# shaderko/velocity-asr

Measured on AMD Instinct MI355X. Metric: audio-sec/sec (RTFx) + frames/s, 5M model batch=32×10s @ 1/2/4/8 MI355X, higher is better.
Workload: dtype f32

## Files before the change

### include/vasr.h

```cpp
#ifndef VASR_H_
#define VASR_H_

#include <stdint.h>

#ifdef __cplusplus
extern "C" {
#endif

#define VASR_ABI_VERSION 21

#define VASR_OK 0
#define VASR_EINVAL (-1)
#define VASR_EUNSUPPORTED (-2)

int vasr_version(void);
const char* vasr_last_error(void);

enum vasr_option {
    VASR_OPT_SCAN_LANES = 0,
    VASR_OPT_SCAN_CHUNK = 1,
    VASR_OPT_TAIL_ROWS = 2,
    VASR_OPT_GEMM_ENGINE = 3,
    VASR_OPT_TAIL_WAVES = 4,
    VASR_OPT_SCAN_SPLIT = 5,
// ... 93 lines not shown

int vasr_ssm_tree_bwd_f32(const float* x, int64_t ld_x, const float* z, int64_t ld_z,
                          const float* dt, int64_t ld_dt, const float* bc, int64_t ld_bc,
                          const float* A, const float* A2, const float* D,
                          const float* g, int64_t ld_g,
                          float* dx, float* ddt, float* dz, float* dB, float* dC,
                          float* dA_part, float* dD_part, float* workspace, int64_t workspace_floats,
                          int B, int L, int Di, int N, void* stream);
int64_t vasr_ssm_tree_bwd_workspace_floats(int B, int L, int Di, int N);

int vasr_ssm_block_tail_f32(const float* g, int64_t ldg, const float* x, int64_t ldx, const uint16_t* wo16,
                            const float* ln_w, const float* ln_b, float ln_eps, const uint16_t* w1_16,
                            const float* b1, const uint16_t* w2_16, const float* b2, float* out, int64_t ldo,
                            int M, int D, int E, void* stream);
int vasr_ssm_block_tail_gated_f32(const float* yd, int64_t ldy, const float* u, int64_t ldu, const uint16_t* wz,
                                  int mode, const float* x, int64_t ldx, const uint16_t* wo16,
                                  const float* ln_w, const float* ln_b, float ln_eps, const uint16_t* w1_16,
                                  const float* b1, const uint16_t* w2_16, const float* b2, float* out, int64_t ldo,
                                  int M, int D, int E, void* stream);
int vasr_ssm_block_tail_bf16(const float* g, int64_t ldg, const float* x, int64_t ldx, const uint16_t* wo16,
                             const float* ln_w, const float* ln_b, float ln_eps, const uint16_t* w1_16,
                             const float* b1, const uint16_t* w2_16, const float* b2, float* out, int64_t ldo,
                             int M, int D, int E, void* stream);
int vasr_ssm_block_tail_gated_bf16(const float* yd, int64_t ldy, const float* u, int64_t ldu, const uint16_t* wz,
                                   int mode, const float* x, int64_t ldx, const uint16_t* wo16,
                                   const float* ln_w, const float* ln_b, float ln_eps, const uint16_t* w1_16,
                                   const float* b1, const uint16_t* w2_16, const float* b2, float* out, int64_t ldo,
                                   int M, int D, int E, void* stream);
int vasr_pack_weights16_bf16(const uint16_t* W, int64_t ldw, int N, int K, uint16_t* out, void* stream);
int64_t vasr_pack_weights16_bf16_elems(int N, int K);
int vasr_split_weights16_bf16x3(const float* W, int64_t ldw, int N, int K, uint16_t* out, void* stream);
int64_t vasr_split_weights16_elems(int N, int K);

int vasr_flac_decode(const uint8_t* data, int64_t n, float* out, int64_t out_cap, int* channels,
                     int* sample_rate, int* bits, int64_t* samples);
int64_t vasr_resample_length(int64_t n, int orig_sr, int new_sr);
int vasr_resample_f32(const float* x, int channels, int64_t n, int64_t ld_x, int orig_sr, int new_sr,
                      float* y, int64_t ld_y);

int vasr_reflect_pad_f32(const float* audio, int64_t ld_audio, float* xp, int64_t ld_out,
                         int B, int S, int pad, void* stream);
int vasr_mel_log_norm_f32(const float* power, int64_t ld_power, int64_t stride_power,
                          const int32_t* fb_rowptr, const int32_t* fb_col, const float* fb_val,
                          float* out, int64_t out_stride, int frame_off, int B, int F, int n_mels,
                          int normalize, float* workspace, void* stream);
int vasr_mel_log_norm_var_f32(const float* power, int64_t ld_power, int64_t stride_power,
                              const int32_t* fb_rowptr, const int32_t* fb_col, const float* fb_val,
                              float* out, int64_t out_stride, int frame_off, int B, int F, int n_mels,
                              int normalize, const int32_t* frames, float* workspace, void* stream);
int64_t vasr_mel_workspace_floats(int B, int F, int n_mels);

int vasr_stft_power_400_f32(const float* audio, int64_t ld_audio, int B, int S, const float* window,
                            float* power, int64_t ldp, int64_t stride_power, void* stream);
int vasr_stft_power_400_var_f32(const float* audio, int64_t ld_audio, int B, int S, const int32_t* samples,
                                const float* window, float* power, int64_t ldp, int64_t stride_power,
                                void* stream);
int vasr_pad_frames_f32(const float* x, float* out, int out_frames, int off,
                        int B, int F, int C, void* stream);

int vasr_adaptive_pool_f32(const float* x, float* out, int B, int L, int C, int K, void* stream);
int vasr_adaptive_pool_var_f32(const float* x, float* out, int B, int L, int C, int K, const int32_t* lens,
                               const int32_t* ks, void* stream);

int vasr_ln_adaptive_pool_f32(const float* x, const float* w, const float* b, float eps, float* out, int B, int L,
                              int C, int K, const int32_t* lens, const int32_t* ks, void* stream);

// ... 72 lines not shown
```

### velocity-asr_amd/velocity_asr/_lib.py

```python

from __future__ import annotations

import ctypes
import os
import re
from typing import Optional

import torch

ABI_VERSION = 21
_HERE = os.path.dirname(os.path.abspath(__file__))
LIB_PATH = os.environ.get("VASR_LIB") or os.path.join(_HERE, "lib", "libvasr_hip.so")
HEADER_PATH = os.path.normpath(os.path.join(_HERE, "..", "..", "include", "vasr.h"))

(EPI_NONE, EPI_GELU, EPI_SOFTPLUS_FROM, EPI_RESIDUAL, EPI_GELU_PE, EPI_PAIR_POWER, EPI_PAIR_FUSION,
 EPI_ARGMAX) = range(8)
OPT_SCAN_LANES, OPT_SCAN_CHUNK, OPT_TAIL_ROWS, OPT_GEMM_ENGINE, OPT_TAIL_WAVES, OPT_SCAN_SPLIT, OPT_DW_ROWS = range(7)

c_i32, c_i64, c_f32, c_p = ctypes.c_int32, ctypes.c_int64, ctypes.c_float, ctypes.c_void_p


class GemmArgs(ctypes.Structure):

    _fields_ = [
# ... 28 lines not shown
    "vasr_add_table_f32": ([c_p, c_p, c_p, ctypes.c_int, ctypes.c_int, ctypes.c_int, c_p], ctypes.c_int),
    "vasr_ln_dwconv_prenorm_f32": ([c_p, c_p, c_p, c_f32, c_p, c_p, c_p, c_p, c_p, c_p] + [ctypes.c_int] * 4
                                   + [c_f32, c_p], ctypes.c_int),
    "vasr_ln_dwconv_f32": ([c_p, c_p, c_p, c_p, c_p, c_p] + [ctypes.c_int] * 4 + [c_f32, c_p], ctypes.c_int),
    "vasr_ssm_scan_f32": ([c_p, c_i64, c_p, c_i64, c_p, c_i64, c_p, c_p, c_p, c_i64] + [ctypes.c_int] * 5 + [c_p],
                          ctypes.c_int),
    "vasr_ssm_scan_chunked_f32": ([c_p, c_i64, c_p, c_i64, c_p, c_i64, c_p, c_p, c_p, c_i64] + [ctypes.c_int] * 5
                                  + [c_p, c_i64, c_p], ctypes.c_int),
    "vasr_ssm_scan_ungated_f32": ([c_p, c_i64, c_p, c_i64, c_p, c_i64, c_p, c_p, c_p, c_i64] + [ctypes.c_int] * 5 + [c_p],
                                  ctypes.c_int),
    "vasr_ssm_scan_workspace_floats": ([ctypes.c_int] * 4, c_i64),
    "vasr_ssm_scan_save_f32": ([c_p, c_i64, c_p, c_i64, c_p, c_i64, c_p, c_p, c_p, c_i64] + [ctypes.c_int] * 5
                               + [c_p, c_i64, c_p], ctypes.c_int),
    "vasr_ssm_scan_checkpoint_floats": ([ctypes.c_int] * 4, c_i64),
    "vasr_ssm_scan_bwd_f32": ([c_p, c_i64, c_p, c_i64, c_p, c_i64, c_p, c_i64, c_p, c_p, c_p, c_p, c_i64] + [c_p] * 9
                              + [c_i64] + [ctypes.c_int] * 4 + [c_p], ctypes.c_int),
    "vasr_ssm_scan_bwd_workspace_floats": ([ctypes.c_int] * 4, c_i64),
    "vasr_ssm_tree_bwd_f32": ([c_p, c_i64, c_p, c_i64, c_p, c_i64, c_p, c_i64, c_p, c_p, c_p, c_p, c_i64] + [c_p] * 8
                              + [c_i64] + [ctypes.c_int] * 4 + [c_p], ctypes.c_int),
    "vasr_ssm_tree_bwd_workspace_floats": ([ctypes.c_int] * 4, c_i64),
    "vasr_ssm_scan_split_selected": ([ctypes.c_int] * 4, ctypes.c_int),
    "vasr_ssm_block_tail_f32": ([c_p, c_i64, c_p, c_i64, c_p, c_p, c_p, c_f32, c_p, c_p, c_p, c_p, c_p, c_i64]
                                + [ctypes.c_int] * 3 + [c_p], ctypes.c_int),
    "vasr_ssm_block_tail_gated_f32": ([c_p, c_i64, c_p, c_i64, c_p, ctypes.c_int, c_p, c_i64, c_p, c_p, c_p, c_f32, c_p,
                                       c_p, c_p, c_p, c_p, c_i64] + [ctypes.c_int] * 3 + [c_p], ctypes.c_int),
    "vasr_ssm_block_tail_gated_bf16": ([c_p, c_i64, c_p, c_i64, c_p, ctypes.c_int, c_p, c_i64, c_p, c_p, c_p, c_f32, c_p,
                                        c_p, c_p, c_p, c_p, c_i64] + [ctypes.c_int] * 3 + [c_p], ctypes.c_int),
    "vasr_ssm_block_tail_bf16": ([c_p, c_i64, c_p, c_i64, c_p, c_p, c_p, c_f32, c_p, c_p, c_p, c_p, c_p, c_i64]
                                 + [ctypes.c_int] * 3 + [c_p], ctypes.c_int),
    "vasr_pack_weights16_bf16": ([c_p, c_i64, ctypes.c_int, ctypes.c_int, c_p, c_p], ctypes.c_int),
    "vasr_pack_weights16_bf16_elems": ([ctypes.c_int, ctypes.c_int], c_i64),
    "vasr_split_weights16_bf16x3": ([c_p, c_i64, ctypes.c_int, ctypes.c_int, c_p, c_p], ctypes.c_int),
    "vasr_split_weights16_elems": ([ctypes.c_int, ctypes.c_int], c_i64),
    "vasr_flac_decode": ([c_p, c_i64, c_p, c_i64, c_p, c_p, c_p, c_p], ctypes.c_int),
    "vasr_resample_length": ([c_i64, ctypes.c_int, ctypes.c_int], c_i64),
    "vasr_resample_f32": ([c_p, ctypes.c_int, c_i64, c_i64, ctypes.c_int, ctypes.c_int, c_p, c_i64], ctypes.c_int),
    "vasr_reflect_pad_f32": ([c_p, c_i64, c_p, c_i64, ctypes.c_int, ctypes.c_int, ctypes.c_int, c_p], ctypes.c_int),
    "vasr_mel_log_norm_f32": ([c_p, c_i64, c_i64, c_p, c_p, c_p, c_p, c_i64] + [ctypes.c_int] * 5 + [c_p, c_p],
                              ctypes.c_int),
    "vasr_mel_workspace_floats": ([ctypes.c_int] * 3, c_i64),
    "vasr_stft_power_400_f32": ([c_p, c_i64, ctypes.c_int, ctypes.c_int, c_p, c_p, c_i64, c_i64, c_p], ctypes.c_int),
    "vasr_stft_power_400_var_f32": ([c_p, c_i64, ctypes.c_int, ctypes.c_int, c_p, c_p, c_p, c_i64, c_i64, c_p],
                                    ctypes.c_int),
    "vasr_mel_log_norm_var_f32": ([c_p, c_i64, c_i64, c_p, c_p, c_p, c_p, c_i64] + [ctypes.c_int] * 5 + [c_p, c_p, c_p],
                                  ctypes.c_int),
    "vasr_adaptive_pool_var_f32": ([c_p, c_p] + [ctypes.c_int] * 4 + [c_p, c_p, c_p], ctypes.c_int),
    "vasr_pooled_attention_var_f32": ([c_p, c_i64, c_p, c_p] + [ctypes.c_int] * 5 + [c_p, c_p], ctypes.c_int),
    "vasr_ctc_collapse_var": ([c_p, ctypes.c_int, ctypes.c_int, c_p, ctypes.c_int, ctypes.c_int, c_p, c_p, c_p, c_p,
                               c_p], ctypes.c_int),
    "vasr_pad_frames_f32": ([c_p, c_p] + [ctypes.c_int] * 5 + [c_p], ctypes.c_int),
    "vasr_ln_adaptive_pool_f32": ([c_p, c_p, c_p, c_f32, c_p] + [ctypes.c_int] * 4 + [c_p, c_p, c_p], ctypes.c_int),
    "vasr_adaptive_pool_f32": ([c_p, c_p] + [ctypes.c_int] * 4 + [c_p], ctypes.c_int),
    "vasr_pooled_attention_f32": ([c_p, c_i64, c_p, c_p] + [ctypes.c_int] * 5 + [c_p], ctypes.c_int),
    "vasr_pooled_attention_bwd_f32": ([c_p, c_i64, c_p, c_p, c_p, c_p, c_p, c_i64] + [ctypes.c_int] * 5 + [c_p, c_p],
                                      ctypes.c_int),
    "vasr_pooled_attention_bwd_workspace_floats": ([ctypes.c_int] * 5, c_i64),
    "vasr_adaptive_pool_bwd_f32": ([c_p, c_p] + [ctypes.c_int] * 4 + [c_p, c_p, c_p], ctypes.c_int),
    "vasr_argmax_f32": ([c_p, c_i64, ctypes.c_int, ctypes.c_int, c_p, c_p], ctypes.c_int),
    "vasr_fakequant_f32": ([c_p, c_i64, c_p, c_i64, ctypes.c_int, ctypes.c_int, c_p, c_p, ctypes.c_int, c_f32, c_f32,
                            c_p], ctypes.c_int),
    "vasr_minmax_f32": ([c_p, c_i64, ctypes.c_int, ctypes.c_int, c_p, c_p, c_p], ctypes.c_int),
    "vasr_argmax_keys": ([c_p, c_i64, ctypes.c_int, ctypes.c_int, c_p, c_p], ctypes.c_int),
    "vasr_ctc_collapse_keys": ([c_p, c_i64] + [ctypes.c_int] * 3 + [c_p, ctypes.c_int, ctypes.c_int] + [c_p] * 6,
                               ctypes.c_int),
    "vasr_ctc_beam_search": ([c_p, c_i64, c_i64] + [ctypes.c_int] * 5 + [c_p] * 5 + [c_p], ctypes.c_int),
    "vasr_ctc_beam_workspace_elems": ([ctypes.c_int, ctypes.c_int], c_i64),
# ... 65 lines not shown
```

### velocity-asr_amd/velocity_asr/attention.py

```python

from __future__ import annotations

import math
import os
from typing import Optional, Sequence, Tuple

import torch
import torch.nn as nn

from . import _lib, ops
from . import quantize as Q
from ._prep import cached
from .ssm import GlobalSSM


def _device_ints(values: Sequence[int], device) -> torch.Tensor:
    return torch.tensor([int(v) for v in values], dtype=torch.int32).to(device)


def _sizes(values, B: int, device) -> Optional[torch.Tensor]:
    if values is None or isinstance(values, torch.Tensor):
        return values
    if len(values) != B:
        raise ValueError(f"expected {B} per-utterance sizes, got {len(values)}")
# ... 219 lines not shown
                raise NotImplementedError("GatedFusion on HIP needs d_model % 32 == 0")
            Wg = Q.effective_weight(gate)
            bg = Q.inner(gate).bias

            def pair(a, b):
                return torch.stack([a.reshape(D // 32, 32, *a.shape[1:]), b.reshape(D // 32, 32, *b.shape[1:])],
                                   1).reshape(2 * D, *a.shape[1:]).contiguous()
            w_local = pair(Wg[:, :D], Q.effective_weight(loc))
            w_glob = pair(Wg[:, D:], Q.effective_weight(glob))
            b_glob = pair(bg, Q.inner(glob).bias)
            qp = None
            if any(Q.act_qparams(m, D) is not None for m in (gate, loc, glob)):
                dev = Wg.device
                qp = torch.cat([pair(Q.act_qparams_or_identity(gate, D, dev), Q.act_qparams_or_identity(glob, D, dev)),
                                Q.act_qparams_or_identity(loc, D, dev)], 0).contiguous()
            return w_local, w_glob, b_glob, qp
        return cached(self, "paired", Q.deps(gate) + Q.deps(loc) + Q.deps(glob), build)

    def _paired_attention(self, mha: "MultiHeadAttention"):
        _, w_glob, b_glob, _ = self._paired()

        def build():
            wo, bo = mha.out_proj.weight, mha.out_proj.bias
            w = (w_glob.detach().double() @ wo.detach().double()).to(w_glob.dtype).contiguous()
            b = (ops.f32(b_glob).double() + w_glob.detach().double() @ ops.f32(bo).detach().double()).float().contiguous()
            return w, b
        return cached(self, "paired_attn", (w_glob, b_glob, mha.out_proj.weight, mha.out_proj.bias), build)

    def composable(self, mha: "MultiHeadAttention") -> bool:
        mods = (mha.out_proj, self.gate_proj[0], self.local_proj, self.global_proj, self.out_proj)
        return (os.environ.get("VASR_ATTN_COMPOSE", "1") != "0" and all(type(m) is nn.Linear for m in mods)
                and len({m.weight.dtype for m in mods}) == 1 and mha.out_proj.bias is not None)

    def forward_attention(self, local_features: torch.Tensor, o: torch.Tensor,
                          mha: "MultiHeadAttention") -> torch.Tensor:
        B, L, D = local_features.shape
        local2 = local_features.reshape(B * L, D)
        w_local, _, _, qp = self._paired()
        w_glob, b_glob = self._paired_attention(mha)
        t1 = ops.gemm(local2, w_local)
        fused = ops.gemm(o, w_glob, b_glob, epilogue=_lib.EPI_PAIR_FUSION, aux=t1,
                         aux2=self.local_proj.bias, n_out=D, qparams=qp)
        out = ops.gemm(fused, self.out_proj.weight, self.out_proj.bias)
        return out.view(B, L, D)

    def _observe(self, local2: torch.Tensor, glob2: torch.Tensor) -> None:
        gate, loc, glob = self.gate_proj[0], self.local_proj, self.global_proj
        D = local2.shape[1]
        Wg = Q.effective_weight(gate)
        if Q.observing(gate):
            t = ops.gemm(local2, Wg[:, :D].contiguous())
            Q.record(gate, ops.gemm(glob2, Wg[:, D:].contiguous(), epilogue=_lib.EPI_RESIDUAL, aux=t)
                     + Q.inner(gate).bias.detach())
        for mod, src in ((loc, local2), (glob, glob2)):
            if Q.observing(mod):
                Q.record(mod, ops.gemm(src, Q.effective_weight(mod), Q.inner(mod).bias))

    def forward(self, local_features: torch.Tensor, global_features: torch.Tensor) -> torch.Tensor:
        B, L, D = local_features.shape
        local2, glob2 = local_features.reshape(B * L, D), global_features.reshape(B * L, D)
        self._observe(local2, glob2)
        w_local, w_glob, b_glob, qp = self._paired()
        t1 = ops.gemm(local2, w_local)
        fused = ops.gemm(glob2, w_glob, b_glob, epilogue=_lib.EPI_PAIR_FUSION, aux=t1,
                         aux2=Q.inner(self.local_proj).bias, n_out=D, qparams=qp)
        wo, bo, qpo = Q.linear_parts(self.out_proj)
        out = ops.gemm(fused, wo, bo, qparams=qpo)
        Q.record(self.out_proj, out)
        return out.view(B, L, D)

    def forward_differentiable(self, local_features: torch.Tensor, global_features: torch.Tensor) -> torch.Tensor:
        F = torch.nn.functional
        gate = self.gate_proj(torch.cat([local_features, global_features], dim=-1))
        local_t = F.linear(local_features, self.local_proj.weight, self.local_proj.bias)
        global_t = F.linear(global_features, self.global_proj.weight, self.global_proj.bias)
        return F.linear(gate * local_t + (1 - gate) * global_t, self.out_proj.weight, self.out_proj.bias)


class HierarchicalGlobalContext(nn.Module):

    def __init__(self, d_model: int = 192, num_heads: int = 4, attention_dim: int = 48, global_ssm_layers: int = 2,
                 global_ssm_state_dim: int = 32, dropout: float = 0.1):
        super().__init__()
        self.pool1 = AdaptivePool(level=1, d_model=d_model)
        self.global_ssm = GlobalSSM(d_model=d_model, num_layers=global_ssm_layers, state_dim=global_ssm_state_dim,
                                    dropout=dropout)
        self.pool2 = AdaptivePool(level=2, d_model=d_model)
        self.cross_attention = MultiHeadAttention(d_model=d_model, num_heads=num_heads, attention_dim=attention_dim,
                                                  dropout=dropout)
        self.norm1 = nn.LayerNorm(d_model)
        self.norm2 = nn.LayerNorm(d_model)
        self.fusion = GatedFusion(d_model=d_model)

    def forward(self, local_features: torch.Tensor, lengths: Optional[Sequence[int]] = None,
                query: Optional[torch.Tensor] = None) -> torch.Tensor:
        x_pool1, pool_size1 = self.pool1(local_features, lengths=lengths)
        gnorm = self.global_ssm.norm
        fold = os.environ.get("VASR_POOL_PRENORM", "0") == "1" and type(gnorm) is nn.LayerNorm
        x_ssm = self.global_ssm(x_pool1, raw=fold)
        x_pool2, pool_size2 = self.pool2(x_ssm, prev_pool_size=pool_size1,
                                         lengths=None if lengths is None else pool_size1,
                                         pre_norm=gnorm if fold else None)
        x_pool2 = ops.layer_norm(x_pool2, self.norm1.weight, self.norm1.bias, self.norm1.eps)
        if query is None:
            query = ops.layer_norm(local_features, self.norm2.weight, self.norm2.bias, self.norm2.eps)
        kl = None if lengths is None else pool_size2
        if self.fusion.composable(self.cross_attention):
            o = self.cross_attention(query=query, key=x_pool2, value=x_pool2, key_lengths=kl, project_out=False)
            return self.fusion.forward_attention(local_features, o, self.cross_attention)
        global_context = self.cross_attention(query=query, key=x_pool2, value=x_pool2, key_lengths=kl)
        return self.fusion(local_features, global_context)

    def forward_differentiable(self, local_features: torch.Tensor,
                               lengths: Optional[Sequence[int]] = None) -> torch.Tensor:
        x_pool1, pool_size1 = self.pool1.forward_differentiable(local_features, lengths=lengths)
        x_ssm = self.global_ssm.forward_differentiable(x_pool1)
        x_pool2, pool_size2 = self.pool2.forward_differentiable(x_ssm, prev_pool_size=pool_size1,
                                                                lengths=None if lengths is None else pool_size1)
        x_pool2 = self.norm1(x_pool2)
        query = self.norm2(local_features)
        global_context = self.cross_attention.forward_differentiable(
            query=query, key=x_pool2, value=x_pool2, key_lengths=None if lengths is None else pool_size2)
        return self.fusion.forward_differentiable(local_features, global_context)
```

### velocity-asr_amd/velocity_asr/model.py

```python

from __future__ import annotations

import math
import os
from dataclasses import dataclass
from typing import Any, Dict, Optional

import torch
import torch.nn as nn

from . import _lib, ops
from . import quantize as Q
from ._prep import cached
from .attention import HierarchicalGlobalContext
from .ssm import LocalSSMProcessor, ScanMode


@dataclass
class VelocityASRConfig:

    mel_bins: int = 80
    d_model: int = 192
    ssm_layers: int = 8
    ssm_state_dim: int = 64
# ... 49 lines not shown
        super().__init__()
        self.conv = nn.Conv1d(in_channels=mel_bins, out_channels=d_model, kernel_size=kernel_size, stride=stride,
                              padding=kernel_size // 2)
        self.pos_encoding = PositionalEncoding2D(d_model=d_model, mel_bins=mel_bins)
        self.norm = nn.LayerNorm(d_model)
        self.activation = nn.GELU()

    def conv_padding(self) -> int:
        return Q.inner(self.conv).padding[0]

    def output_length(self, frames: int) -> int:
        c = Q.inner(self.conv)
        k, s, p = c.kernel_size[0], c.stride[0], c.padding[0]
        return (frames + 2 * p - k) // s + 1

    def forward(self, mel_spectrogram: torch.Tensor, raw: bool = False) -> torch.Tensor:
        D = Q.inner(self.conv).out_channels
        L = self.output_length(mel_spectrogram.shape[1])
        if Q.observing(self.conv):
            Q.record(self.conv, Q.conv1d_rows(self.conv, mel_spectrogram))
        x = Q.conv1d_rows(self.conv, mel_spectrogram, epilogue=_lib.EPI_GELU_PE, aux=self.pos_encoding.table(L),
                          ld_aux=D)
        if raw:
            return x
        return ops.layer_norm(x, self.norm.weight, self.norm.bias, self.norm.eps)


class CTCOutputHead(nn.Module):

    def __init__(self, d_model: int = 192, vocab_size: int = 50000, dropout: float = 0.1):
        super().__init__()
        self.proj = nn.Sequential(nn.LayerNorm(d_model), nn.Dropout(dropout), nn.Linear(d_model, vocab_size))

    def forward(self, x: torch.Tensor) -> torch.Tensor:
        B, L, D = x.shape
        ln = self.proj[0]
        w, b, qp = Q.linear_parts(self.proj[2])
        logits = ops.gemm(x.reshape(B * L, D), w, b, qparams=qp, ln=(ln.weight, ln.bias, ln.eps))
        Q.record(self.proj[2], logits)
        return logits.view(B, L, w.shape[0])

    def argmax(self, x: torch.Tensor) -> torch.Tensor:
        B, L, D = x.shape
        ln = self.proj[0]
        w, b, qp = Q.linear_parts(self.proj[2])
        return ops.gemm_argmax(x.reshape(B * L, D), w, b, qparams=qp, ln=(ln.weight, ln.bias, ln.eps)).view(B, L)

    def greedy(self, x: torch.Tensor, blank: int = 0, out=None, rows=None):
        B, L, D = x.shape
        ln = self.proj[0]
        w, b, qp = Q.linear_parts(self.proj[2])
        toks, lens, _, _ = ops.gemm_ctc_greedy(x.reshape(B * L, D), w, b, B, blank, qparams=qp,
                                               ln=(ln.weight, ln.bias, ln.eps), out=out, frames=rows)
        return toks, lens


class VELOCITYASR(nn.Module):

    def __init__(self, config: Optional[VelocityASRConfig] = None):
        super().__init__()
        if config is None:
            config = VelocityASRConfig()
        self.config = config
        self.temporal_binding = TemporalBindingLayer(mel_bins=config.mel_bins, d_model=config.d_model)
        self.local_ssm = LocalSSMProcessor(d_model=config.d_model, num_layers=config.ssm_layers,
                                           state_dim=config.ssm_state_dim, expand_ratio=config.ssm_expand_ratio,
                                           kernel_size=config.ssm_kernel_size, dropout=config.dropout,
                                           use_checkpoint=config.gradient_checkpointing, scan_mode=config.scan_mode)
        self.global_context = HierarchicalGlobalContext(d_model=config.d_model, num_heads=config.attention_heads,
                                                        attention_dim=config.attention_dim,
                                                        global_ssm_layers=config.global_ssm_layers,
                                                        global_ssm_state_dim=config.global_ssm_state_dim,
                                                        dropout=config.dropout)
        self.ctc_head = CTCOutputHead(d_model=config.d_model, vocab_size=config.vocab_size, dropout=config.dropout)
        self._init_weights()

    def _init_weights(self):
        for module in self.modules():
            if isinstance(module, nn.Linear):
                nn.init.xavier_uniform_(module.weight)
                if module.bias is not None:
                    nn.init.zeros_(module.bias)
            elif isinstance(module, nn.Conv1d):
                nn.init.kaiming_normal_(module.weight, mode="fan_out", nonlinearity="relu")
                if module.bias is not None:
                    nn.init.zeros_(module.bias)
            elif isinstance(module, nn.LayerNorm):
                nn.init.ones_(module.weight)
                nn.init.zeros_(module.bias)

    def _token_lengths(self, frames, n_frames: int):
        if frames is None:
            return None
        frames = [int(f) for f in frames]
        if not all(1 <= f <= n_frames for f in frames):
            raise ValueError(f"frames: each utterance needs 1..{n_frames} frames, got {frames}")
        return [self.temporal_binding.output_length(f) for f in frames]

    def _local_global(self, mel: torch.Tensor, lengths):
        gc, tb = self.global_context, self.temporal_binding
        pre = None
        if os.environ.get("VASR_TB_PRENORM", "1") != "0" and type(tb.norm) is nn.LayerNorm:
            x, pre = tb(mel, raw=True), tb.norm
        else:
            x = tb(mel)
        if os.environ.get("VASR_LN_PAIR", "1") != "0" and type(gc.norm2) is nn.LayerNorm \
                and type(self.local_ssm.norm) is nn.LayerNorm:
            local, query = self.local_ssm.forward_pair(x, gc.norm2, pre_norm=pre)
            return local, gc(local, lengths=lengths, query=query)
        local = self.local_ssm(x, pre_norm=pre)
        return local, gc(local, lengths=lengths)

    def forward(self, mel_spectrogram: torch.Tensor, return_features: bool = False, frames=None):
        if mel_spectrogram.device.type != "cuda":
            _lib.require_device()
            raise RuntimeError("velocity_asr (MI355X build): move the model and input to the HIP device "
                               "(model.to('cuda'), mel.to('cuda')); there is no CPU execution path")
        mel = mel_spectrogram.to(torch.float32)
        lengths = self._token_lengths(frames, mel.shape[1])
        with torch.no_grad():
            if return_features:
                x = self.temporal_binding(mel)
                local_features = self.local_ssm(x)
                fused_features = self.global_context(local_features, lengths=lengths)
            else:
                local_features, fused_features = self._local_global(mel, lengths)
            logits = self.ctc_head(fused_features)
        if return_features:
            return logits, {"temporal_binding": x, "local_features": local_features,
                            "fused_features": fused_features}
        return logits

    def token_ids(self, mel_spectrogram: torch.Tensor, frames=None) -> torch.Tensor:
        if mel_spectrogram.device.type != "cuda":
            _lib.require_device()
            raise RuntimeError("velocity_asr (MI355X build): token_ids needs HIP tensors")
        lengths = self._token_lengths(frames, mel_spectrogram.shape[1])
        with torch.no_grad():
            x = self._local_global(mel_spectrogram.to(torch.float32), lengths)[1]
            return self.ctc_head.argmax(x)

    def greedy_token_ids(self, mel_spectrogram: torch.Tensor, frames=None, blank: int = 0, out=None, rows=None):
        if mel_spectrogram.device.type != "cuda":
            _lib.require_device()
            raise RuntimeError("velocity_asr (MI355X build): greedy_token_ids needs HIP tensors")
        lengths = self._token_lengths(frames, mel_spectrogram.shape[1])
        with torch.no_grad():
            x = self._local_global(mel_spectrogram.to(torch.float32), lengths)[1]
            return self.ctc_head.greedy(x, blank, out=out, rows=rows)

    def get_output_length(self, input_length: int) -> int:
        return (input_length + 1) // 2

    @classmethod
    def from_pretrained(cls, model_name_or_path: str, quantized: bool = False, **kwargs) -> "VELOCITYASR":
        if not os.path.exists(model_name_or_path):
            raise NotImplementedError("Model hub download not yet implemented. "
                                      "Please provide a local path to the checkpoint.")
        checkpoint = torch.load(model_name_or_path, map_location="cpu", weights_only=True)
        if "config" in checkpoint:
            config = VelocityASRConfig.from_dict(checkpoint["config"])
        else:
            config = VelocityASRConfig()
        model = cls(config)
        if "model_state_dict" in checkpoint:
            model.load_state_dict(checkpoint["model_state_dict"])
        else:
            model.load_state_dict(checkpoint)
        return model

    def save_pretrained(self, save_path: str):
        d = os.path.dirname(save_path)
        if d:
            os.makedirs(d, exist_ok=True)
        c = self.config
        checkpoint = {
            "config": {
                "mel_bins": c.mel_bins, "d_model": c.d_model, "ssm_layers": c.ssm_layers,
                "ssm_state_dim": c.ssm_state_dim, "ssm_expand_ratio": c.ssm_expand_ratio,
                "ssm_kernel_size": c.ssm_kernel_size, "global_ssm_layers": c.global_ssm_layers,
                "global_ssm_state_dim": c.global_ssm_state_dim, "attention_heads": c.attention_heads,
                "attention_dim": c.attention_dim, "vocab_size": c.vocab_size, "dropout": c.dropout,
# ... 10 lines not shown
```

### velocity-asr_amd/velocity_asr/ops.py

```python

from __future__ import annotations

import math
import os
import weakref
from typing import Optional, Tuple

import torch

from . import _lib as L
from ._lib import GemmArgs, check, ptr, stream_of

LOG2E = 1.4426950408889634

_timing = None


class kernel_timer:

    def __init__(self, *names):
        self.names = set(names)
        self.records = {n: [] for n in names}

    def __enter__(self):
# ... 134 lines not shown
          "vasr_pack_weights16_bf16")
    key = id(w)
    _splits16[key] = (weakref.ref(w, _dropper(_splits16, key)), sig, packed)
    return packed


def ssm_block_tail(g: torch.Tensor, x: torch.Tensor, wo: torch.Tensor, ln_w: torch.Tensor, ln_b: torch.Tensor,
                   ln_eps: float, w1: torch.Tensor, b1: torch.Tensor, w2: torch.Tensor, b2: torch.Tensor,
                   out: Optional[torch.Tensor] = None) -> torch.Tensor:
    bf16 = wo.dtype == torch.bfloat16
    if bf16:
        if not (w1.dtype == w2.dtype == torch.bfloat16):
            raise TypeError("ssm_block_tail: mixed weight dtypes")
        ln_w, ln_b, b1, b2 = f32(ln_w), f32(ln_b), f32(b1), f32(b2)
    for n, t in (("g", g), ("x", x), ("ln_w", ln_w), ("ln_b", ln_b), ("b1", b1), ("b2", b2)) + (
            () if bf16 else (("wo", wo), ("w1", w1), ("w2", w2))):
        _cuda_f32(f"ssm_block_tail.{n}", t)
    M, E, ldg = _rows("ssm_block_tail.g", g)
    Mx, D, ldx = _rows("ssm_block_tail.x", x)
    if Mx != M or tuple(wo.shape) != (D, E) or tuple(w1.shape) != (E, D) or tuple(w2.shape) != (D, E):
        raise ValueError("ssm_block_tail: inconsistent shapes")
    if out is None:
        out = torch.empty((M, D), device=g.device, dtype=torch.float32)
    _, _, ldo = _rows("ssm_block_tail.out", out)
    prep = pack_weights16 if bf16 else split_weights16
    fn = "vasr_ssm_block_tail_bf16" if bf16 else "vasr_ssm_block_tail_f32"
    ev = _t0("ssm_tail")
    check(getattr(L.lib(), fn)(g.data_ptr(), ldg, x.data_ptr(), ldx, prep(wo).data_ptr(), ln_w.contiguous().data_ptr(),
                               ln_b.contiguous().data_ptr(), float(ln_eps), prep(w1).data_ptr(),
                               b1.contiguous().data_ptr(), prep(w2).data_ptr(), b2.contiguous().data_ptr(),
                               out.data_ptr(), ldo, M, D, E, stream_of(g)), fn)
    _t1("ssm_tail", ev, dict(M=M, D=D, E=E))
    return out


def pack_bf16(w: torch.Tensor) -> torch.Tensor:
    N, K, ldw = _rows("pack.w", w)
    sig = (w.data_ptr(), w._version, N, K, ldw)
    ent = _splits.get(id(w))
    if ent is not None and ent[0]() is w and ent[1] == sig:
        return ent[2]
    packed = torch.empty(int(L.lib().vasr_pack_weights_bf16_elems(N, K)), device=w.device, dtype=torch.int16)
    check(L.lib().vasr_pack_weights_bf16(w.data_ptr(), ldw, N, K, packed.data_ptr(), stream_of(w)),
          "vasr_pack_weights_bf16")
    key = id(w)
    _splits[key] = (weakref.ref(w, _dropper(_splits, key)), sig, packed)
    return packed


def _linear(args: GemmArgs, w: torch.Tensor, stream) -> None:
    if w.dtype == torch.bfloat16:
        check(L.lib().vasr_linear_bf16(args, pack_bf16(w).data_ptr(), stream), "vasr_linear_bf16")
    else:
        check(L.lib().vasr_linear_x3_f32(args, split_weights(w).data_ptr(), stream), "vasr_linear_x3_f32")


def gemm_tile(M: int, N: int, K: int, *, batch: int = 1, epilogue: int = L.EPI_NONE, bf16: bool = False) -> int:
    k = L.lib().vasr_gemm_tile(int(M), int(N), int(K), int(batch), int(epilogue), int(bool(bf16)))
    check(min(k, 0), "vasr_gemm_tile")
    return k


def _ln_prologue(a: torch.Tensor, ln) -> torch.Tensor:
    if ln is None:
        return a
    ln_w, ln_b, eps = ln
# ... 863 lines not shown
```

Before: 165,000.

## Fuse gated-fusion GEMMs, output projection and CTC head LayerNorm into one kernel

Adds a HIP kernel that, per row tile, computes the local and global projection GEMMs with split-bf16 (3-plane) MFMA, applies the sigmoid gate blend, runs the output projection, and applies the CTC head's LayerNorm, writing the normalized features directly. The Python path routes the global-context fusion through this kernel when shapes match (d_model 192, attention dim 48) and tells the CTC head to skip its own LayerNorm. This removes several kernel launches and round-trips of intermediates through global memory. In exchange it adds a large specialized kernel that holds weight prefetch rings in registers and may have limited occupancy with one block per CU.

```diff
diff --git a/include/vasr.h b/include/vasr.h
--- a/include/vasr.h
+++ b/include/vasr.h
@@ -149,6 +149,11 @@
 int vasr_split_weights16_bf16x3(const float* W, int64_t ldw, int N, int K, uint16_t* out, void* stream);
 int64_t vasr_split_weights16_elems(int N, int K);
 
+int vasr_fusion_tail_f32(const float* local, int64_t ldl, const float* o, int64_t ldo, const uint16_t* w_local,
+                         const uint16_t* w_glob, const float* b_glob, const float* b_local, const uint16_t* w_out,
+                         const float* b_out, const float* ln_w, const float* ln_b, float ln_eps, float* y,
+                         int64_t ldy, float* out, int64_t ldout, int M, int D, int A, int rows, void* stream);
+
 int vasr_flac_decode(const uint8_t* data, int64_t n, float* out, int64_t out_cap, int* channels,
                      int* sample_rate, int* bits, int64_t* samples);
 int64_t vasr_resample_length(int64_t n, int orig_sr, int new_sr);
diff --git a/velocity-asr_amd/csrc/fusion_tail.hip b/velocity-asr_amd/csrc/fusion_tail.hip
--- /dev/null
+++ b/velocity-asr_amd/csrc/fusion_tail.hip
@@ -0,0 +1,310 @@
+#include "ssm_fused.h"
+
+namespace vasr {
+namespace {
+
+using namespace fused;
+typedef float floatx16 __attribute__((ext_vector_type(16)));
+
+constexpr int TA = 48;
+constexpr int OW = 64;
+constexpr int XLD = 200;
+constexpr int NST = 27;
+constexpr int SG = 3, ST = 15;
+
+#ifndef VASR_FT_PD32
+#define VASR_FT_PD32 2
+#endif
+#ifndef VASR_FT_PD64
+#define VASR_FT_PD64 1
+#endif
+
+struct FusionParams {
+    const float* local;
+    int64_t ldl;
+    const float* o;
+    int64_t ldo;
+    const uint16_t* wl;
+    const uint16_t* wg;
+    const float* bg;
+    const float* bl;
+    const uint16_t* wo;
+    const float* bo;
+    const float* ln_w;
+    const float* ln_b;
+    float ln_eps;
+    float* y;
+    int64_t ldy;
+    float* out;
+    int64_t ldout;
+    int M;
+};
+
+template <int RT>
+struct FusionCtx {
+    static constexpr int NWV = 6 * RT;
+    static constexpr int ROWS = 32 * RT;
+    static constexpr int PD = RT == 1 ? VASR_FT_PD32 : VASR_FT_PD64;
+    static constexpr int RING = PD + 1;
+    static constexpr int PL = ROWS * TD * 2;
+    static constexpr int PO = ROWS * OW * 2;
+    const FusionParams& P;
+    char* A;
+    char* O;
+    const float* sb;
+    float* xs;
+    int lane, w, row, zh, m0;
+    floatx16 g[2], t[2], oc;
+    bf16x8 a[2][3];
+    bf16x8 wf[RING][2][3];
+};
+
+template <int S, int RT>
+__device__ __forceinline__ void load_w(FusionCtx<RT>& c) {
+    constexpr int slot = S % FusionCtx<RT>::RING;
+    if constexpr (S < ST) {
+        const char* W = reinterpret_cast<const char*>(S < SG ? c.P.wg : c.P.wl);
+        constexpr int KS = S < SG ? 4 : TD / 16, ks = S < SG ? S : S - SG;
+#pragma unroll
+        for (int j = 0; j < 2; ++j)
+#pragma unroll
+            for (int pl = 0; pl < 3; ++pl)
+                c.wf[slot][j][pl] = *reinterpret_cast<const bf16x8*>(
+                    W + ((int64_t)((2 * c.w + j) * KS + ks) * 3 + pl) * 1024 + c.lane * 16);
+    } else {
+        const char* W = reinterpret_cast<const char*>(c.P.wo);
+#pragma unroll
+        for (int pl = 0; pl < 3; ++pl)
+            c.wf[slot][0][pl] = *reinterpret_cast<const bf16x8*>(
+                W + ((int64_t)(c.w * (TD / 16) + (S - ST)) * 3 + pl) * 1024 + c.lane * 16);
+    }
+}
+
+template <int S, int RT>
+__device__ __forceinline__ void load_first(FusionCtx<RT>& c) {
+    load_w<S, RT>(c);
+    if constexpr (S + 1 < FusionCtx<RT>::PD) load_first<S + 1, RT>(c);
+}
+
+template <int S, int RT>
+__device__ __forceinline__ void read_a(FusionCtx<RT>& c, bf16x8 (&a)[3]) {
+    using Ctx = FusionCtx<RT>;
+    if constexpr (S < SG) {
+#pragma unroll
+        for (int pl = 0; pl < 3; ++pl)
+            a[pl] = *reinterpret_cast<const bf16x8*>(c.O + pl * Ctx::PO + c.row * OW * 2 +
+                                                     (((2 * S + c.zh) ^ ((c.row >> 1) & 7)) << 4));
+    } else {
+        constexpr int ks = S < ST ? S - SG : S - ST;
+#pragma unroll
+        for (int pl = 0; pl < 3; ++pl)
+            a[pl] = *reinterpret_cast<const bf16x8*>(c.A + pl * Ctx::PL + c.row * TD * 2 +
+                                                     (((2 * ks + c.zh) ^ (c.row & 7)) << 4));
+    }
+}
+
+__device__ __forceinline__ void blend_store4(char* plane0, int plane_bytes, int off, const float (&tg)[4],
+                                             const float (&tl)[4], const float (&gg)[4], const float (&gl)[4],
+                                             const float4& bg, const float4& bgl, const float4& b2) {
+#pragma clang fp contract(off)
+    typedef __bf16 bf16x4 __attribute__((ext_vector_type(4)));
+    const float bgv[4] = {bg.x, bg.y, bg.z, bg.w}, bglv[4] = {bgl.x, bgl.y, bgl.z, bgl.w};
+    const float b2v[4] = {b2.x, b2.y, b2.z, b2.w};
+    bf16x4 hi, mid, lo;
+#pragma unroll
+    for (int i = 0; i < 4; ++i) {
+        const float gp = (tg[i] + gg[i]) + bgv[i];
+        const float lt = tl[i] + b2v[i];
+        const float gt = gl[i] + bglv[i];
+        const float gate = sigmoid_fast(gp);
+        const float v = gate * lt + (1.0f - gate) * gt;
+        hi[i] = (__bf16)v;
+        const float r1 = v - (float)hi[i];
+        mid[i] = (__bf16)r1;
+        lo[i] = (__bf16)(r1 - (float)mid[i]);
+    }
+    *reinterpret_cast<bf16x4*>(plane0 + off) = hi;
+    *reinterpret_cast<bf16x4*>(plane0 + plane_bytes + off) = mid;
+    *reinterpret_cast<bf16x4*>(plane0 + 2 * plane_bytes + off) = lo;
+}
+
+__device__ __forceinline__ void mac_pair_t(floatx16 (&acc)[2], const bf16x8 (&w)[2][3], const bf16x8 (&a)[3]) {
+    constexpr int pa[6] = {2, 0, 1, 1, 0, 0}, pw[6] = {0, 2, 1, 0, 1, 0};
+#pragma unroll
+    for (int p = 0; p < 6; ++p)
+#pragma unroll
+        for (int j = 0; j < 2; ++j) acc[j] = __builtin_amdgcn_mfma_f32_32x32x16_bf16(w[j][pw[p]], a[pa[p]], acc[j], 0, 0, 0);
+}
+
+__device__ __forceinline__ floatx16 mac_chunk(floatx16 acc, const bf16x8 (&a)[3], const bf16x8 (&w)[3]) {
+    constexpr int pa[6] = {2, 0, 1, 1, 0, 0}, pw[6] = {0, 2, 1, 0, 1, 0};
+#pragma unroll
+    for (int p = 0; p < 6; ++p) acc = __builtin_amdgcn_mfma_f32_32x32x16_bf16(a[pa[p]], w[pw[p]], acc, 0, 0, 0);
+    return acc;
+}
+
+template <int S, int RT>
+__device__ __forceinline__ void fusion_step(FusionCtx<RT>& c) {
+    using Ctx = FusionCtx<RT>;
+    constexpr int PD = Ctx::PD;
+    if constexpr (S + PD < NST) load_w<S + PD, RT>(c);
+    __builtin_amdgcn_sched_barrier(0);
+    if constexpr (S == 0 || S == ST) read_a<S, RT>(c, c.a[S & 1]);
+    if constexpr (S + 1 < NST && S + 1 != ST) read_a<S + 1, RT>(c, c.a[(S + 1) & 1]);
+    __builtin_amdgcn_sched_barrier(0);
+    const bf16x8(&a)[3] = c.a[S & 1];
+    const bf16x8(&w)[2][3] = c.wf[S % Ctx::RING];
+    if constexpr (S < SG) {
+        mac_pair_t(c.g, w, a);
+    } else if constexpr (S < ST) {
+        if constexpr (S == SG) {
+#pragma unroll
+            for (int i = 0; i < 16; ++i) c.t[0][i] = c.t[1][i] = 0.f;
+        }
+        mac_pair_t(c.t, w, a);
+    } else {
+        if constexpr (S == ST) {
+#pragma unroll
+            for (int i = 0; i < 16; ++i) c.oc[i] = 0.f;
+        }
+        c.oc = mac_chunk(c.oc, a, w[0]);
+    }
+
+    if constexpr (S == ST - 1) {
+        lds_barrier();
+#pragma unroll
+        for (int j = 0; j < 4; ++j) {
+            const int cc = 8 * j + 4 * c.zh;
+            const float4 bg = *reinterpret_cast<const float4*>(c.sb + 64 * c.w + cc);
+            const float4 bgl = *reinterpret_cast<const float4*>(c.sb + 64 * c.w + 32 + cc);
+            const float4 b2 = *reinterpret_cast<const float4*>(c.sb + 2 * TD + 32 * c.w + cc);
+            const float tg[4] = {c.t[0][4 * j], c.t[0][4 * j + 1], c.t[0][4 * j + 2], c.t[0][4 * j + 3]};
+            const float tl[4] = {c.t[1][4 * j], c.t[1][4 * j + 1], c.t[1][4 * j + 2], c.t[1][4 * j + 3]};
+            const float gg[4] = {c.g[0][4 * j], c.g[0][4 * j + 1], c.g[0][4 * j + 2], c.g[0][4 * j + 3]};
+            const float gl[4] = {c.g[1][4 * j], c.g[1][4 * j + 1], c.g[1][4 * j + 2], c.g[1][4 * j + 3]};
+            blend_store4(c.A, Ctx::PL, poff<TD>(c.row, 32 * c.w + cc), tg, tl, gg, gl, bg, bgl, b2);
+        }
+        lds_barrier();
+    }
+    if constexpr (S + 1 < NST) fusion_step<S + 1, RT>(c);
+}
+
+template <int RT>
+__global__ __launch_bounds__(384 * RT, 1) void fusion_tail_kernel(FusionParams P) {
+    using Ctx = FusionCtx<RT>;
+    constexpr int NT = 64 * Ctx::NWV;
+    __shared__ __attribute__((aligned(16))) char A[3 * Ctx::PL];
+    __shared__ __attribute__((aligned(16))) char O[3 * Ctx::PO];
+    __shared__ __attribute__((aligned(16))) float xs[Ctx::ROWS * XLD];
+    __shared__ __attribute__((aligned(16))) float sb[4 * TD];
+    Ctx c{P, A, O, sb, xs};
+    c.lane = threadIdx.x & 63;
+    const int wave = __builtin_amdgcn_readfirstlane((int)threadIdx.x >> 6);
+    c.w = wave % 6;
+    c.row = 32 * (wave / 6) + (c.lane & 31);
+    c.zh = c.lane >> 5;
+    c.m0 = blockIdx.x * Ctx::ROWS;
+    load_first<0, RT>(c);
+    __builtin_amdgcn_sched_barrier(0);
+    constexpr int UNITS = Ctx::ROWS * (TD / 8);
+    static_assert(UNITS % NT == 0, "whole staging rounds");
+#pragma unroll
+    for (int k = 0; k < UNITS / NT; ++k) {
+        const int u = threadIdx.x + NT * k;
+        const int rr = u / (TD / 8), ch = u - rr * (TD / 8);
+        const float* src = P.local + (int64_t)min(c.m0 + rr, P.M - 1) * P.ldl + 8 * ch;
+        const float4 v0 = *reinterpret_cast<const float4*>(src);
+        const float4 v1 = *reinterpret_cast<const float4*>(src + 4);
+        split_store8<3>(A, Ctx::PL, rr * TD * 2 + ((ch ^ (rr & 7)) << 4), v0, v1);
+    }
+    if (threadIdx.x < Ctx::ROWS * (TA / 8)) {
+        const int rr = threadIdx.x / (TA / 8), ch = threadIdx.x - rr * (TA / 8);
+        const float* src = P.o + (int64_t)min(c.m0 + rr, P.M - 1) * P.ldo + 8 * ch;
+        const float4 v0 = *reinterpret_cast<const float4*>(src);
+        const float4 v1 = *reinterpret_cast<const float4*>(src + 4);
+        split_store8<3>(O, Ctx::PO, rr * OW * 2 + ((ch ^ ((rr >> 1) & 7)) << 4), v0, v1);
+    }
+    for (int i = threadIdx.x; i < 4 * TD; i += NT)
+        sb[i] = i < 2 * TD ? P.bg[i] : i < 3 * TD ? P.bl[i - 2 * TD] : P.bo[i - 3 * TD];
+#pragma unroll
+    for (int i = 0; i < 16; ++i) {
+        c.g[0][i] = 0.f;
+        c.g[1][i] = 0.f;
+    }
+    lds_barrier();
+    fusion_step<0, RT>(c);
+    const int ln = (int)__builtin_amdgcn_mbcnt_hi(~0u, __builtin_amdgcn_mbcnt_lo(~0u, 0u));
+    {
+        const int col = 32 * c.w + (ln & 31);
+        const int r0 = 32 * (wave / 6) + 4 * (ln >> 5);
+        const float bo = sb[3 * TD + col];
+#pragma unroll
+        for (int i = 0; i < 16; ++i) {
+            const int rr = r0 + (i & 3) + 8 * (i >> 2);
+            const float v = c.oc[i] + bo;
+            xs[rr * XLD + col] = v;
+            if (P.out && c.m0 + rr < P.M) P.out[(int64_t)(c.m0 + rr) * P.ldout + col] = v;
+        }
+    }
+    lds_barrier();
+    float lw[3], lb[3];
+#pragma unroll
+    for (int i = 0; i < 3; ++i) {
+        lw[i] = P.ln_w[ln + 64 * i];
+        lb[i] = P.ln_b[ln + 64 * i];
+    }
+    for (int rr = wave; rr < Ctx::ROWS && c.m0 + rr < P.M; rr += Ctx::NWV) {
+        float v[3];
+        float s = 0.f;
+#pragma unroll
+        for (int i = 0; i < 3; ++i) {
+            v[i] = xs[rr * XLD + ln + 64 * i];
+            s += v[i];
+        }
+        const float mean = wave_sum(s) / (float)TD;
+        float q = 0.f;
+#pragma unroll
+        for (int i = 0; i < 3; ++i) {
+            const float d = v[i] - mean;
+            q = __builtin_fmaf(d, d, q);
+        }
+        const float var = wave_sum(q) / (float)TD;
+        const float rstd = 1.0f / sqrtf(var + P.ln_eps);
+        float* yr = P.y + (int64_t)(c.m0 + rr) * P.ldy;
+#pragma unroll
+        for (int i = 0; i < 3; ++i) yr[ln + 64 * i] = __builtin_fmaf((v[i] - mean) * rstd, lw[i], lb[i]);
+    }
+}
+
+int fusion_rows(int M) { return M > 8192 ? 64 : 32; }
+
+}
+}
+
+VASR_API int vasr_fusion_tail_f32(const float* local, int64_t ldl, const float* o, int64_t ldo,
+                                  const uint16_t* w_local, const uint16_t* w_glob, const float* b_glob,
+                                  const float* b_local, const uint16_t* w_out, const float* b_out, const float* ln_w,
+                                  const float* ln_b, float ln_eps, float* y, int64_t ldy, float* out, int64_t ldout,
+                                  int M, int D, int A, int rows, void* stream) {
+    using namespace vasr;
+    VASR_CHECK_ARG(local && o && w_local && w_glob && b_glob && b_local && w_out && b_out && ln_w && ln_b && y,
+                   "vasr_fusion_tail_f32: null pointer");
+    VASR_CHECK_ARG(D == TD && A == TA, "vasr_fusion_tail_f32: built for d_model %d, attention dim %d (got %d, %d)", TD, TA,
+                   D, A);
+    VASR_CHECK_ARG(M >= 0 && ldl >= D && ldo >= A && ldy >= D && (!out || ldout >= D) && ldl % 4 == 0 && ldo % 4 == 0,
+                   "vasr_fusion_tail_f32: bad shape M=%d ldl=%lld ldo=%lld ldy=%lld ldout=%lld", M, (long long)ldl,
+                   (long long)ldo, (long long)ldy, (long long)ldout);
+    VASR_CHECK_ARG(((reinterpret_cast<uintptr_t>(local) | reinterpret_cast<uintptr_t>(o) |
+                     reinterpret_cast<uintptr_t>(w_local) | reinterpret_cast<uintptr_t>(w_glob) |
+                     reinterpret_cast<uintptr_t>(w_out)) & 15) == 0,
+                   "vasr_fusion_tail_f32: local, o and the weight planes must be 16-byte aligned");
+    VASR_CHECK_ARG(rows == 0 || rows == 32 || rows == 64, "vasr_fusion_tail_f32: rows must be 0 (automatic), 32 or 64");
+    if (M == 0) return VASR_OK;
+    const FusionParams p{local, ldl, o, ldo, w_local, w_glob, b_glob, b_local, w_out, b_out, ln_w, ln_b, ln_eps,
+                         y, ldy, out, ldout, M};
+    const int r = rows ? rows : fusion_rows(M);
+    const dim3 grid((unsigned)((M + r - 1) / r));
+    if (r == 64) hipLaunchKernelGGL((fusion_tail_kernel<2>), grid, dim3(768), 0, as_stream(stream), p);
+    else hipLaunchKernelGGL((fusion_tail_kernel<1>), grid, dim3(384), 0, as_stream(stream), p);
+    return launch_status("vasr_fusion_tail_f32");
+}
diff --git a/velocity-asr_amd/velocity_asr/_lib.py b/velocity-asr_amd/velocity_asr/_lib.py
--- a/velocity-asr_amd/velocity_asr/_lib.py
+++ b/velocity-asr_amd/velocity_asr/_lib.py
@@ -84,6 +84,8 @@
     "vasr_pack_weights16_bf16_elems": ([ctypes.c_int, ctypes.c_int], c_i64),
     "vasr_split_weights16_bf16x3": ([c_p, c_i64, ctypes.c_int, ctypes.c_int, c_p, c_p], ctypes.c_int),
     "vasr_split_weights16_elems": ([ctypes.c_int, ctypes.c_int], c_i64),
+    "vasr_fusion_tail_f32": ([c_p, c_i64, c_p, c_i64] + [c_p] * 8 + [c_f32, c_p, c_i64, c_p, c_i64]
+                             + [ctypes.c_int] * 4 + [c_p], ctypes.c_int),
     "vasr_flac_decode": ([c_p, c_i64, c_p, c_i64, c_p, c_p, c_p, c_p], ctypes.c_int),
     "vasr_resample_length": ([c_i64, ctypes.c_int, ctypes.c_int], c_i64),
     "vasr_resample_f32": ([c_p, ctypes.c_int, c_i64, c_i64, ctypes.c_int, ctypes.c_int, c_p, c_i64], ctypes.c_int),
diff --git a/velocity-asr_amd/velocity_asr/attention.py b/velocity-asr_amd/velocity_asr/attention.py
--- a/velocity-asr_amd/velocity_asr/attention.py
+++ b/velocity-asr_amd/velocity_asr/attention.py
@@ -275,12 +275,23 @@
         return (os.environ.get("VASR_ATTN_COMPOSE", "1") != "0" and all(type(m) is nn.Linear for m in mods)
                 and len({m.weight.dtype for m in mods}) == 1 and mha.out_proj.bias is not None)
 
+    def fusable(self, mha: "MultiHeadAttention", head_norm) -> bool:
+        return (os.environ.get("VASR_FUSION_TAIL", "1") != "0" and type(head_norm) is nn.LayerNorm
+                and self.composable(mha) and self.out_proj.weight.dtype == torch.float32
+                and head_norm.weight is not None and head_norm.weight.dtype == torch.float32
+                and head_norm.bias is not None and tuple(self.out_proj.weight.shape) == (192, 192)
+                and mha.attention_dim == 48 and self.out_proj.bias is not None and self.local_proj.bias is not None)
+
     def forward_attention(self, local_features: torch.Tensor, o: torch.Tensor,
-                          mha: "MultiHeadAttention") -> torch.Tensor:
+                          mha: "MultiHeadAttention", head_norm: Optional[nn.LayerNorm] = None) -> torch.Tensor:
         B, L, D = local_features.shape
         local2 = local_features.reshape(B * L, D)
         w_local, _, _, qp = self._paired()
         w_glob, b_glob = self._paired_attention(mha)
+        if head_norm is not None:
+            y, _ = ops.fusion_tail(local2, o, w_local, w_glob, b_glob, self.local_proj.bias, self.out_proj.weight,
+                                   self.out_proj.bias, head_norm.weight, head_norm.bias, head_norm.eps)
+            return y.view(B, L, D)
         t1 = ops.gemm(local2, w_local)
         fused = ops.gemm(o, w_glob, b_glob, epilogue=_lib.EPI_PAIR_FUSION, aux=t1,
                          aux2=self.local_proj.bias, n_out=D, qparams=qp)
@@ -336,7 +347,7 @@
         self.fusion = GatedFusion(d_model=d_model)
 
     def forward(self, local_features: torch.Tensor, lengths: Optional[Sequence[int]] = None,
-                query: Optional[torch.Tensor] = None) -> torch.Tensor:
+                query: Optional[torch.Tensor] = None, head_norm: Optional[nn.LayerNorm] = None):
         x_pool1, pool_size1 = self.pool1(local_features, lengths=lengths)
         gnorm = self.global_ssm.norm
         fold = os.environ.get("VASR_POOL_PRENORM", "0") == "1" and type(gnorm) is nn.LayerNorm
@@ -350,9 +361,13 @@
         kl = None if lengths is None else pool_size2
         if self.fusion.composable(self.cross_attention):
             o = self.cross_attention(query=query, key=x_pool2, value=x_pool2, key_lengths=kl, project_out=False)
-            return self.fusion.forward_attention(local_features, o, self.cross_attention)
-        global_context = self.cross_attention(query=query, key=x_pool2, value=x_pool2, key_lengths=kl)
-        return self.fusion(local_features, global_context)
+            if head_norm is not None and self.fusion.fusable(self.cross_attention, head_norm):
+                return self.fusion.forward_attention(local_features, o, self.cross_attention, head_norm), True
+            out = self.fusion.forward_attention(local_features, o, self.cross_attention)
+        else:
+            global_context = self.cross_attention(query=query, key=x_pool2, value=x_pool2, key_lengths=kl)
+            out = self.fusion(local_features, global_context)
+        return out if head_norm is None else (out, False)
 
     def forward_differentiable(self, local_features: torch.Tensor,
                                lengths: Optional[Sequence[int]] = None) -> torch.Tensor:
diff --git a/velocity-asr_amd/velocity_asr/model.py b/velocity-asr_amd/velocity_asr/model.py
--- a/velocity-asr_amd/velocity_asr/model.py
+++ b/velocity-asr_amd/velocity_asr/model.py
@@ -105,26 +105,27 @@
         super().__init__()
         self.proj = nn.Sequential(nn.LayerNorm(d_model), nn.Dropout(dropout), nn.Linear(d_model, vocab_size))
 
-    def forward(self, x: torch.Tensor) -> torch.Tensor:
-        B, L, D = x.shape
+    def _ln(self, normalized: bool):
         ln = self.proj[0]
+        return None if normalized else (ln.weight, ln.bias, ln.eps)
+
+    def forward(self, x: torch.Tensor, normalized: bool = False) -> torch.Tensor:
+        B, L, D = x.shape
         w, b, qp = Q.linear_parts(self.proj[2])
-        logits = ops.gemm(x.reshape(B * L, D), w, b, qparams=qp, ln=(ln.weight, ln.bias, ln.eps))
+        logits = ops.gemm(x.reshape(B * L, D), w, b, qparams=qp, ln=self._ln(normalized))
         Q.record(self.proj[2], logits)
         return logits.view(B, L, w.shape[0])
 
-    def argmax(self, x: torch.Tensor) -> torch.Tensor:
-        B, L, D = x.shape
-        ln = self.proj[0]
+    def argmax(self, x: torch.Tensor, normalized: bool = False) -> torch.Tensor:
+        B, L, D = x.shape
         w, b, qp = Q.linear_parts(self.proj[2])
-        return ops.gemm_argmax(x.reshape(B * L, D), w, b, qparams=qp, ln=(ln.weight, ln.bias, ln.eps)).view(B, L)
-
-    def greedy(self, x: torch.Tensor, blank: int = 0, out=None, rows=None):
-        B, L, D = x.shape
-        ln = self.proj[0]
+        return ops.gemm_argmax(x.reshape(B * L, D), w, b, qparams=qp, ln=self._ln(normalized)).view(B, L)
+
+    def greedy(self, x: torch.Tensor, blank: int = 0, out=None, rows=None, normalized: bool = False):
+        B, L, D = x.shape
         w, b, qp = Q.linear_parts(self.proj[2])
         toks, lens, _, _ = ops.gemm_ctc_greedy(x.reshape(B * L, D), w, b, B, blank, qparams=qp,
-                                               ln=(ln.weight, ln.bias, ln.eps), out=out, frames=rows)
+                                               ln=self._ln(normalized), out=out, frames=rows)
         return toks, lens
 
 
@@ -172,6 +173,7 @@
 
     def _local_global(self, mel: torch.Tensor, lengths):
         gc, tb = self.global_context, self.temporal_binding
+        hn = self.ctc_head.proj[0]
         pre = None
         if os.environ.get("VASR_TB_PRENORM", "1") != "0" and type(tb.norm) is nn.LayerNorm:
             x, pre = tb(mel, raw=True), tb.norm
@@ -180,9 +182,9 @@
         if os.environ.get("VASR_LN_PAIR", "1") != "0" and type(gc.norm2) is nn.LayerNorm \
                 and type(self.local_ssm.norm) is nn.LayerNorm:
             local, query = self.local_ssm.forward_pair(x, gc.norm2, pre_norm=pre)
-            return local, gc(local, lengths=lengths, query=query)
+            return (local,) + gc(local, lengths=lengths, query=query, head_norm=hn)
         local = self.local_ssm(x, pre_norm=pre)
-        return local, gc(local, lengths=lengths)
+        return (local,) + gc(local, lengths=lengths, head_norm=hn)
 
     def forward(self, mel_spectrogram: torch.Tensor, return_features: bool = False, frames=None):
         if mel_spectrogram.device.type != "cuda":
@@ -192,13 +194,14 @@
         mel = mel_spectrogram.to(torch.float32)
         lengths = self._token_lengths(frames, mel.shape[1])
         with torch.no_grad():
+            normalized = False
             if return_features:
                 x = self.temporal_binding(mel)
                 local_features = self.local_ssm(x)
                 fused_features = self.global_context(local_features, lengths=lengths)
             else:
-                local_features, fused_features = self._local_global(mel, lengths)
-            logits = self.ctc_head(fused_features)
+                local_features, fused_features, normalized = self._local_global(mel, lengths)
+            logits = self.ctc_head(fused_features, normalized=normalized)
         if return_features:
             return logits, {"temporal_binding": x, "local_features": local_features,
                             "fused_features": fused_features}
@@ -210,8 +213,8 @@
             raise RuntimeError("velocity_asr (MI355X build): token_ids needs HIP tensors")
         lengths = self._token_lengths(frames, mel_spectrogram.shape[1])
         with torch.no_grad():
-            x = self._local_global(mel_spectrogram.to(torch.float32), lengths)[1]
-            return self.ctc_head.argmax(x)
+            _, x, normalized = self._local_global(mel_spectrogram.to(torch.float32), lengths)
+            return self.ctc_head.argmax(x, normalized=normalized)
 
     def greedy_token_ids(self, mel_spectrogram: torch.Tensor, frames=None, blank: int = 0, out=None, rows=None):
         if mel_spectrogram.device.type != "cuda":
@@ -219,8 +222,8 @@
             raise RuntimeError("velocity_asr (MI355X build): greedy_token_ids needs HIP tensors")
         lengths = self._token_lengths(frames, mel_spectrogram.shape[1])
         with torch.no_grad():
-            x = self._local_global(mel_spectrogram.to(torch.float32), lengths)[1]
-            return self.ctc_head.greedy(x, blank, out=out, rows=rows)
+            _, x, normalized = self._local_global(mel_spectrogram.to(torch.float32), lengths)
+            return self.ctc_head.greedy(x, blank, out=out, rows=rows, normalized=normalized)
 
     def get_output_length(self, input_length: int) -> int:
         return (input_length + 1) // 2
diff --git a/velocity-asr_amd/velocity_asr/ops.py b/velocity-asr_amd/velocity_asr/ops.py
--- a/velocity-asr_amd/velocity_asr/ops.py
+++ b/velocity-asr_amd/velocity_asr/ops.py
@@ -190,6 +190,31 @@
                                out.data_ptr(), ldo, M, D, E, stream_of(g)), fn)
     _t1("ssm_tail", ev, dict(M=M, D=D, E=E))
     return out
+
+
+def fusion_tail(local: torch.Tensor, o: torch.Tensor, w_local: torch.Tensor, w_glob: torch.Tensor,
+                b_glob: torch.Tensor, b_local: torch.Tensor, w_out: torch.Tensor, b_out: torch.Tensor,
+                ln_w: torch.Tensor, ln_b: torch.Tensor, ln_eps: float, *, want_out: bool = False, rows: int = 0):
+    for n, t in (("local", local), ("o", o), ("w_local", w_local), ("w_glob", w_glob), ("b_glob", b_glob),
+                 ("b_local", b_local), ("w_out", w_out), ("b_out", b_out), ("ln_w", ln_w), ("ln_b", ln_b)):
+        _cuda_f32(f"fusion_tail.{n}", t)
+    M, D, ldl = _rows("fusion_tail.local", local)
+    Mo, A, ldo = _rows("fusion_tail.o", o)
+    if Mo != M or tuple(w_local.shape) != (2 * D, D) or tuple(w_glob.shape) != (2 * D, A) \
+            or tuple(w_out.shape) != (D, D) or b_glob.numel() != 2 * D \
+            or any(t.numel() != D for t in (b_local, b_out, ln_w, ln_b)):
+        raise ValueError("fusion_tail: inconsistent shapes")
+    y = torch.empty((M, D), device=local.device, dtype=torch.float32)
+    out = torch.empty((M, D), device=local.device, dtype=torch.float32) if want_out else None
+    ev = _t0("fusion_tail")
+    check(L.lib().vasr_fusion_tail_f32(local.data_ptr(), ldl, o.data_ptr(), ldo, split_weights(w_local).data_ptr(),
+                                       split_weights(w_glob).data_ptr(), b_glob.contiguous().data_ptr(),
+                                       b_local.contiguous().data_ptr(), split_weights(w_out).data_ptr(),
+                                       b_out.contiguous().data_ptr(), ln_w.contiguous().data_ptr(),
+                                       ln_b.contiguous().data_ptr(), float(ln_eps), y.data_ptr(), D, ptr(out), D,
+                                       M, D, A, int(rows), stream_of(local)), "vasr_fusion_tail_f32")
+    _t1("fusion_tail", ev, dict(M=M, D=D, A=A))
+    return y, out
 
 
 def pack_bf16(w: torch.Tensor) -> torch.Tensor:
```

Result: faster. 167,400, median of 6 (+1.5%).
